# safe-autonomous-systems/fluidgym

Measured on NVIDIA B200. Metric: env-steps/sec (solver steps x envs), higher is better.
Workload: dtype f32

## Files before the change

fluidgym_b200/csrc/piso_b200.cu:

```cuda
#include <cuda_runtime.h>
#include <cooperative_groups.h>
#include <stdint.h>
#include <stdio.h>
#include <stdlib.h>
#include <string.h>
#include <math.h>
#include <new>

#include "fluidgym_b200.h"

namespace cg = cooperative_groups;

static thread_local char g_err[512] = "";
static int set_err(int code, const char *msg, cudaError_t ce = cudaSuccess) {
    if (ce != cudaSuccess) snprintf(g_err, sizeof(g_err), "%s: %s", msg, cudaGetErrorString(ce));
    else snprintf(g_err, sizeof(g_err), "%s", msg);
    return code;
}
extern "C" const char *fgb_last_error(void) { return g_err; }
extern "C" int fgb_version(void) { return 1; }

#define LAUNCH_CHECK(name)                                                       \
    do {                                                                         \
        cudaError_t e_ = cudaGetLastError();                                     \
// ... 1221 lines not shown
            const int nb = ok ? t.nbr[ff * N + g] : -1;
            if (flags & 1) co[k][ff] = (ok && nb >= 0) ? off[(int)t.rev[ff * N + g] * N + nb] : 0.f;
            else co[k][ff] = (ok && nb >= 0) ? off[ff * N + g] : 0.f;
            const int gi = nb >= 0 ? nb : (ok ? g : start);
            const int c = gi / per;
            if (PUSH) na[k][ff] = vs_addr + 4u * (uint32_t)(ok ? t.cg_slot[ff * N + g] : 0);
            else na[k][ff] = mapa_u32(vs_addr + 4u * (uint32_t)(gi - c * per), (uint32_t)c);
        }
    }
    const uint32_t peer_red = mapa_u32(red_addr, (uint32_t)(lane < CS ? lane : 0));
    const uint32_t peer_mb = mapa_u32(mb_addr, (uint32_t)(lane < CS ? lane : 0));
    cluster_sync_all();

    uint32_t rcount = 0;
    uint32_t pphase = 0;
    auto cluster_sum = [&](float a0) -> float {
        const uint32_t w = rcount & 1u, par = (rcount >> 1) & 1u;
#pragma unroll
        for (int o = 16; o > 0; o >>= 1) a0 += __shfl_xor_sync(0xffffffffu, a0, o);
        if (lane < CS) st_async_f32(peer_red + 4u * (w * NP + rank * NW + (uint32_t)warp), a0, peer_mb + 8u * w);
        mbar_wait(mb_addr + 8u * w, par);
        const float *rp = red + w * NP;
        float s0 = 0.f;
#pragma unroll
        for (int q = 0; q < (NP + 31) / 32; ++q) s0 += (lane + 32 * q < NP) ? rp[lane + 32 * q] : 0.f;
#pragma unroll
        for (int o = 16; o > 0; o >>= 1) s0 += __shfl_xor_sync(0xffffffffu, s0, o);
        if (threadIdx.x == 0) mbar_arrive_expect_tx(mb_addr + 8u * w, NP * 4);
        ++rcount;
        return s0;
    };
    auto publish = [&]() {
        __syncthreads();
        if (PUSH) {
            for (int e = threadIdx.x; e < n_exp; e += T) {
                const uint2 ex = exps[e];
                st_async_f32(ex.y, ld_shared_f32(vs_addr + (ex.x & 0xffffffu)), mapa_u32(mb_addr + 16, ex.x >> 24));
            }
        } else if (threadIdx.x < CS) mbar_arrive_remote_release(mapa_u32(mb_addr + 16, threadIdx.x));
    };
    auto acquire_p = [&]() {
        mbar_wait(mb_addr + 16, pphase); pphase ^= 1u;
        if (PUSH && threadIdx.x == 0) mbar_arrive_expect_tx(mb_addr + 16, halo_bytes);
    };
    auto apply = [&](int k) -> float {
        float s = cd[k] * vs[threadIdx.x + k * T];
#pragma unroll
        for (int ff = 0; ff < 4; ++ff) s += co[k][ff] * (PUSH ? ld_shared_f32(na[k][ff]) : ld_dsmem_f32(na[k][ff]));
        return s;
    };
    auto load_f = [&](int k) -> float { const int l = threadIdx.x + k * T; return l < cnt ? f[start + l] : 0.f; };

    float nz = 0.f;
#pragma unroll
    for (int k = 0; k < CPT; ++k) nz += (load_f(k) != 0.f) ? 1.f : 0.f;
    const float nzt = cluster_sum(nz);
    int used = -1; float fin = 0.f;
    if (!(nzt > 0.f)) {
#pragma unroll
        for (int k = 0; k < CPT; ++k) xr[k] = 0.f;
    } else {
        if (!zero_init) {
#pragma unroll
            for (int k = 0; k < CPT; ++k) vs[threadIdx.x + k * T] = xr[k];
            publish(); acquire_p();
#pragma unroll
            for (int k = 0; k < CPT; ++k) rr[k] = load_f(k) - apply(k);
            (void)cluster_sum(0.f);
        } else {
#pragma unroll
            for (int k = 0; k < CPT; ++k) rr[k] = load_f(k);
        }
        float a0 = 0.f;
#pragma unroll
        for (int k = 0; k < CPT; ++k) { const int l = threadIdx.x + k * T; vs[l] = rr[k]; bs[l] = xr[k]; a0 += rr[k] * rr[k]; }
        publish();
        float rho = cluster_sum(a0);
        float bestc = 0.f, lastc = 0.f; int best_it = -1, rising = 0;
        bool take_best = false;
        float pk[CPT], apk[CPT];
        for (int i = 0; i < maxit; ++i) {
            if (reset_steps > 0 && (i + 1) % reset_steps == 0) {
                acquire_p();
                (void)cluster_sum(0.f);
#pragma unroll
                for (int k = 0; k < CPT; ++k) vs[threadIdx.x + k * T] = xr[k];
                publish(); acquire_p();
#pragma unroll
                for (int k = 0; k < CPT; ++k) rr[k] = load_f(k) - apply(k);
                (void)cluster_sum(0.f);
                a0 = 0.f;
#pragma unroll
                for (int k = 0; k < CPT; ++k) { vs[threadIdx.x + k * T] = rr[k]; a0 += rr[k] * rr[k]; }
                publish();
                rho = cluster_sum(a0);
            }
            acquire_p();
            a0 = 0.f;
#pragma unroll
            for (int k = 0; k < CPT; ++k) {
                apk[k] = apply(k);
                pk[k] = vs[threadIdx.x + k * T];
                a0 += pk[k] * apk[k];
            }
            const float pap = cluster_sum(a0);
            const float alpha = rho / pap;
            a0 = 0.f;
#pragma unroll
            for (int k = 0; k < CPT; ++k) {
                xr[k] += alpha * pk[k];
                rr[k] -= alpha * apk[k];
                a0 += rr[k] * rr[k];
            }
            const float rr2 = cluster_sum(a0);
            const float crit = sqrtf(rr2) * norm;
            int stop = isfinite(crit) ? 0 : 1;
            used = i; fin = crit;
            if (!stop) {
                if (i == 0 || crit < bestc) {
                    bestc = crit; best_it = i;
#pragma unroll
                    for (int k = 0; k < CPT; ++k) bs[threadIdx.x + k * T] = xr[k];
                }
                if (i > 0 && crit >= lastc) ++rising; else rising = 0;
                lastc = crit;
                if (crit < tol) stop = 1;
                else if (i == maxit - 1 || rising >= 100) stop = 2;
            }
            asm volatile("" : "+r"(stop));
            if (stop) { take_best = stop == 2; break; }
            const float beta = rr2 / rho;
            rho = rr2;
#pragma unroll
            for (int k = 0; k < CPT; ++k) vs[threadIdx.x + k * T] = rr[k] + beta * pk[k];
            publish();
        }
        if (take_best) {
#pragma unroll
            for (int k = 0; k < CPT; ++k) xr[k] = bs[threadIdx.x + k * T];
            used = best_it; fin = bestc;
        }
    }
    float sx = 0.f;
#pragma unroll
    for (int k = 0; k < CPT; ++k) sx += xr[k];
    const float mean = (flags & 2) ? 0.f : cluster_sum(sx) / (float)N;
    if (mean_out && threadIdx.x == 0 && rank == 0) mean_out[b] = mean;
#pragma unroll
    for (int k = 0; k < CPT; ++k) { const int l = threadIdx.x + k * T; if (l < cnt) xo[start + l] = xr[k] - mean; }
    if (threadIdx.x == 0 && rank == 0) { iters[b * 8 + 2 + slot] = used; resid[b * 8 + 2 + slot] = fin; iter_total[b * 2] += (unsigned long long)(used + 1); }
    cluster_sync_all();
}

template <int T, int CPT, int CS, int MINB>
__global__ void __launch_bounds__(T, MINB) k_cg_strip(Tab t, const float *__restrict__ Poff, const float *__restrict__ Pdiag,
                                                    const float *__restrict__ Rhs, float *__restrict__ Xout,
                                                    int maxit, float tol, int zero_init, int reset_steps, int slot,
                                                    const int32_t *__restrict__ active, int32_t *__restrict__ iters,
                                                    float *__restrict__ resid, unsigned long long *__restrict__ iter_total,
                                                    int flags, float *__restrict__ mean_out, float *__restrict__ best) {
    static_assert(T % 32 == 0, "whole warps only: every warp contributes exactly one partial sum per exchange");
    constexpr int NW = T / 32;
    const int b = blockIdx.x / CS;
    uint32_t rank;
    asm volatile("mov.u32 %0, %%cluster_ctarank;" : "=r"(rank));
    if (active && !active[b]) return;
    extern __shared__ __align__(16) float smem[];
    const int N = t.N, SL = t.st_slots, G = t.st_gmax;
    float4 *co4 = reinterpret_cast<float4 *>(smem);
    float *cdg = smem + 4 * CPT * T;
    float *vs = cdg + CPT * T;
    float *rs = vs + SL;
    float *red = rs + G;
    float *wpart = red + 2 * CS + (2 * CS & 1 ? 1 : 0);
    unsigned long long *mb = (unsigned long long *)(wpart + 2 * NW + (2 * NW & 1 ? 1 : 0));
    uint2 *rex = (uint2 *)(mb + 4);
    uint2 *lex = rex + t.st_remax;
    const float *off = Poff + (size_t)b * 4 * N, *dg = Pdiag + (size_t)b * N, *f = Rhs + (size_t)b * N;
    float *xo = Xout + (size_t)b * N;
    const float norm = 1.0f / sqrtf((float)N);
    const uint32_t red_addr = smem_u32(red), mb_addr = smem_u32(mb), rs_addr = smem_u32(rs);
    const int tid = threadIdx.x, lane = tid & 31, warp = tid >> 5;

    const int4 th0 = reinterpret_cast<const int4 *>(t.st_thread)[((size_t)rank * T + tid) * 2];
    const int4 th1 = reinterpret_cast<const int4 *>(t.st_thread)[((size_t)rank * T + tid) * 2 + 1];
    const int S = th0.y;
    float *vp = vs + th0.x;
    const int re_off = th0.w & 0xffff, re_cnt = (th0.w >> 16) & 0xff;
    const int n_lex = t.st_cnt[4 * rank + 2];
    const float *rgp = rs + th1.y;
    const uint32_t rm = (uint32_t)th1.z;
    const int32_t *cellp = t.st_cell + ((size_t)rank * T + tid) * CPT;
    float *bestp = best + ((size_t)b * CS + rank) * T * CPT + tid;
    const uint32_t bytesA = CS * 4u, bytesB = CS * 4u + 4u * (uint32_t)t.st_cnt[4 * rank];
    if (tid == 0) {
        mbar_init(mb_addr, 1); mbar_init(mb_addr + 8, 1);
        mbar_init(mb_addr + 16, NW); mbar_init(mb_addr + 24, NW);
        asm volatile("fence.mbarrier_init.release.cluster;" ::: "memory");
        mbar_arrive_expect_tx(mb_addr, bytesA);
        mbar_arrive_expect_tx(mb_addr + 8, bytesB);
    }
    for (int e = tid; e < t.st_cnt[4 * rank + 1]; e += T) {
        const int32_t a = t.st_rexp[((size_t)rank * t.st_remax + e) * 2], d = t.st_rexp[((size_t)rank * t.st_remax + e) * 2 + 1];
        rex[e] = make_uint2((uint32_t)a, mapa_u32(rs_addr + 4u * (uint32_t)d, (uint32_t)a >> 8));
    }
    for (int e = tid; e < n_lex; e += T)
        lex[e] = make_uint2((uint32_t)t.st_lexp[((size_t)rank * t.st_lemax + e) * 2], (uint32_t)t.st_lexp[((size_t)rank * t.st_lemax + e) * 2 + 1]);
    for (int i = tid; i < SL + G; i += T) vs[i] = 0.f;

    float x[CPT], r[CPT], ap[CPT];
#pragma unroll
    for (int k = 0; k < CPT; ++k) {
        const int c = cellp[k];
        const bool real = c >= 0;
        const int g = real ? c : (c <= -2 ? -2 - c : 0);
        float co[4];
#pragma unroll
        for (int d = 0; d < 4; ++d) {
            const int ff = (th0.z >> (2 * d)) & 3;
            const int nb = real ? t.nbr[ff * N + g] : -1;
            if (flags & 1) co[d] = nb >= 0 ? off[(int)t.rev[ff * N + g] * N + nb] : 0.f;
            else co[d] = nb >= 0 ? off[ff * N + g] : 0.f;
        }
        co4[k * T + tid] = make_float4(co[0], co[1], co[2], co[3]);
        cdg[k * T + tid] = real ? dg[g] : 0.f;
        x[k] = (c != -1 && !zero_init) ? xo[g] : 0.f;
        r[k] = real ? f[g] : 0.f;
        ap[k] = 0.f;
    }
    const uint32_t peer_red = mapa_u32(red_addr, (uint32_t)(lane < CS ? lane : 0));
    const uint32_t peer_mb = mapa_u32(mb_addr, (uint32_t)(lane < CS ? lane : 0));
    cluster_sync_all();

    uint32_t parA = 0, parB = 0;
    auto exchange = [&](float a0, const uint32_t which, uint32_t &par, const uint32_t bytes) -> float {
#pragma unroll
        for (int o = 16; o > 0; o >>= 1) a0 += __shfl_xor_sync(0xffffffffu, a0, o);
        if (lane == 0) {
            wpart[which * NW + warp] = a0;
            asm volatile("mbarrier.arrive.release.cta.shared::cta.b64 _, [%0];" ::"r"(mb_addr + 16u + 8u * which) : "memory");
        }
        if (warp == 0) {
            mbar_wait_sleep(mb_addr + 16u + 8u * which, par);
            float s1 = lane < NW ? wpart[which * NW + lane] : 0.f;
#pragma unroll
            for (int o = 16; o > 0; o >>= 1) s1 += __shfl_xor_sync(0xffffffffu, s1, o);
            if (lane < CS) st_async_f32(peer_red + 4u * (which * CS + rank), s1, peer_mb + 8u * which);
        }
        mbar_wait_sleep(mb_addr + 8u * which, par); par ^= 1u;
        float s0 = 0.f;
#pragma unroll
        for (int q = 0; q < CS; ++q) s0 += red[which * CS + q];
        if (tid == 0) mbar_arrive_expect_tx(mb_addr + 8u * which, bytes);
        return s0;
    };
    auto row_of = [&](const float (&v)[CPT], int kk) -> float {
        float s = v[0];
#pragma unroll
        for (int k = 1; k < CPT; ++k) s = (kk == k) ? v[k] : s;
        return s;
    };
    auto spmv = [&]() -> float {
        float a0 = 0.f, a1 = 0.f;
        float vsouth = vp[-S], vc = vp[0];
#pragma unroll
        for (int k = 0; k < CPT; ++k) {
            const float *row = vp + k * S;
            const float vnorth = row[S];
            const float4 o = co4[k * T + tid];
            float s = cdg[k * T + tid] * vc;
            s = fmaf(o.x, row[-1], s);
            s = fmaf(o.y, row[1], s);
            s = fmaf(o.z, vsouth, s);
            s = fmaf(o.w, vnorth, s);
            ap[k] = s;
            if (k & 1) a1 = fmaf(vc, s, a1); else a0 = fmaf(vc, s, a0);
            vsouth = vc; vc = vnorth;
        }
        return a0 + a1;
    };
    auto mirror_local_ghosts = [&]() {
        __syncthreads();
        if (n_lex) {
            for (int e = tid; e < n_lex; e += T) { const uint2 ex = lex[e]; vs[ex.y] = vs[ex.x]; }
            __syncthreads();
        }
    };
    auto publish_x = [&]() {
#pragma unroll
        for (int k = 0; k < CPT; ++k) vp[k * S] = x[k];
        mirror_local_ghosts();
    };
    auto new_direction = [&](float beta) {
        if (rm) {
            int n = 0;
#pragma unroll
            for (int k = 0; k < CPT; ++k) if (rm & (1u << k)) r[k] = rgp[n++];
        }
#pragma unroll
        for (int k = 0; k < CPT; ++k) ap[k] = vp[k * S];
#pragma unroll
        for (int k = 0; k < CPT; ++k) vp[k * S] = fmaf(beta, ap[k], r[k]);
        if (rm) {
#pragma unroll
            for (int k = 0; k < CPT; ++k) if (rm & (1u << k)) r[k] = 0.f;
        }
        mirror_local_ghosts();
    };
    auto residual_norm2 = [&]() -> float {
        for (int j = 0; j < re_cnt; ++j) {
            const uint2 ex = rex[re_off + j];
            st_async_f32(ex.y, row_of(r, (int)(ex.x & 0xff)), mapa_u32(mb_addr + 8, ex.x >> 8));
        }
        float a0 = 0.f, a1 = 0.f;
#pragma unroll
        for (int k = 0; k < CPT; k += 2) { a0 = fmaf(r[k], r[k], a0); if (k + 1 < CPT) a1 = fmaf(r[k + 1], r[k + 1], a1); }
        return exchange(a0 + a1, 1u, parB, bytesB);
    };

    float nz = 0.f;
#pragma unroll
    for (int k = 0; k < CPT; ++k) nz += (r[k] != 0.f) ? 1.f : 0.f;
    const float nzt = exchange(nz, 0u, parA, bytesA);
    int used = -1; float fin = 0.f;
    bool solved = false;
    if (!(nzt > 0.f)) {
#pragma unroll
        for (int k = 0; k < CPT; ++k) x[k] = 0.f;
    } else {
        solved = true;
        if (!zero_init) {
            publish_x();
            (void)spmv();
#pragma unroll
            for (int k = 0; k < CPT; ++k) r[k] -= ap[k];
            __syncthreads();
        }
#pragma unroll
        for (int k = 0; k < CPT; ++k) bestp[k * T] = x[k];
        float rho = residual_norm2();
        new_direction(0.f);
        float bestc = 0.f, lastc = 0.f; int best_it = -1, rising = 0;
        bool take_best = false;
        int until_reset = reset_steps > 0 ? reset_steps - 1 : -1;
        for (int i = 0; i < maxit; ++i) {
            if (until_reset == 0) {
                until_reset = reset_steps;
                (void)exchange(0.f, 0u, parA, bytesA);
                publish_x();
                (void)spmv();
#pragma unroll
                for (int k = 0; k < CPT; ++k) { const int c = cellp[k]; r[k] = (c >= 0 ? f[c] : 0.f) - ap[k]; }
                __syncthreads();
                rho = residual_norm2();
                new_direction(0.f);
            }
            --until_reset;
            const float pap = exchange(spmv(), 0u, parA, bytesA);
            const float alpha = rho / pap;
#pragma unroll
            for (int k = 0; k < CPT; ++k) {
                x[k] = fmaf(alpha, vp[k * S], x[k]);
                r[k] = fmaf(-alpha, ap[k], r[k]);
            }
            const float rr2 = residual_norm2();
            const float crit = sqrtf(rr2) * norm;
            int stop = isfinite(crit) ? 0 : 1;
            used = i; fin = crit;
            if (!stop) {
                if (i == 0 || crit < bestc) {
                    bestc = crit; best_it = i;
#pragma unroll
                    for (int k = 0; k < CPT; ++k) bestp[k * T] = x[k];
                }
                if (i > 0 && crit >= lastc) ++rising; else rising = 0;
                lastc = crit;
                if (crit < tol) stop = 1;
                else if (i == maxit - 1 || rising >= 100) stop = 2;
            }
            asm volatile("" : "+r"(stop));
            if (stop) { take_best = stop == 2; break; }
            const float beta = rr2 / rho;
            rho = rr2;
            new_direction(beta);
        }
        if (take_best) {
#pragma unroll
            for (int k = 0; k < CPT; ++k) x[k] = bestp[k * T];
            used = best_it; fin = bestc;
        }
    }
    float mean = 0.f;
    if (solved && !(flags & 2)) {
        float sx = 0.f;
#pragma unroll
        for (int k = 0; k < CPT; ++k) sx += (cellp[k] >= 0) ? x[k] : 0.f;
        mean = exchange(sx, 0u, parA, bytesA) / (float)N;
    }
    if (mean_out && tid == 0 && rank == 0) mean_out[b] = mean;
#pragma unroll
    for (int k = 0; k < CPT; ++k) { const int c = cellp[k]; if (c >= 0) xo[c] = x[k] - mean; }
    if (tid == 0 && rank == 0) { iters[b * 8 + 2 + slot] = used; resid[b * 8 + 2 + slot] = fin; iter_total[b * 2] += (unsigned long long)(used + 1); }
    cluster_sync_all();
}

template <int E> struct EnvTag { static constexpr int value = E; };

template <int T, int CPT, int CS>
__global__ void __launch_bounds__(T, 1) k_cg_strip2(Tab t, const float *__restrict__ Poff, const float *__restrict__ Pdiag,
                                                    const float *__restrict__ Rhs, float *__restrict__ Xout, int B,
                                                    int maxit, float tol, int zero_init, int reset_steps, int slot,
                                                    const int32_t *__restrict__ active, int32_t *__restrict__ iters,
                                                    float *__restrict__ resid, unsigned long long *__restrict__ iter_total,
                                                    int flags, float *__restrict__ mean_out, float *__restrict__ best) {
    static_assert(T % 32 == 0, "whole warps only");
    constexpr int NW = T / 32;
    constexpr uint32_t FULL = 0xffffffffu;
    const int b0 = 2 * (int)(blockIdx.x / CS);
    uint32_t rank;
    asm volatile("mov.u32 %0, %%cluster_ctarank;" : "=r"(rank));
    bool on[2];
    on[0] = !active || active[b0];
    on[1] = b0 + 1 < B && (!active || active[b0 + 1]);
    if (!on[0] && !on[1]) return;
    extern __shared__ __align__(16) float smem[];
    const int N = t.N, SL = t.st_slots, G = t.st_gmax;
    const int ENVF = (5 * CPT * T + SL + G + 2 * CS + 2 * NW + 3) & ~3;
    unsigned long long *mb = (unsigned long long *)(smem + 2 * ENVF);
    unsigned int *cnt = (unsigned int *)(mb + 4);
    uint2 *rex = (uint2 *)(cnt + 4);
    uint2 *lex = rex + t.st_remax;
    const float norm = 1.0f / sqrtf((float)N);
    const uint32_t mb_addr = smem_u32(mb);
    const int tid = threadIdx.x, lane = tid & 31, warp = tid >> 5;

    const int4 th0 = reinterpret_cast<const int4 *>(t.st_thread)[((size_t)rank * T + tid) * 2];
    const int4 th1 = reinterpret_cast<const int4 *>(t.st_thread)[((size_t)rank * T + tid) * 2 + 1];
    const int S = th0.y;
    const int vp_off = 5 * CPT * T + th0.x;
    const int re_off = th0.w & 0xffff, re_cnt = (th0.w >> 16) & 0xff;
    const int n_lex = t.st_cnt[4 * rank + 2];
    const int rg_off = 5 * CPT * T + SL + th1.y;
    const uint32_t rm = (uint32_t)th1.z;
    const int32_t *cellp = t.st_cell + ((size_t)rank * T + tid) * CPT;
    const uint32_t bytesA = CS * 4u, bytesB = CS * 4u + 4u * (uint32_t)t.st_cnt[4 * rank];
    if (tid == 0) {
#pragma unroll
        for (int e = 0; e < 2; ++e) {
            mbar_init(mb_addr + 16u * e, 1); mbar_init(mb_addr + 16u * e + 8u, 1);
            cnt[2 * e] = 0u; cnt[2 * e + 1] = 0u;
        }
        asm volatile("fence.mbarrier_init.release.cluster;" ::: "memory");
#pragma unroll
        for (int e = 0; e < 2; ++e) { mbar_arrive_expect_tx(mb_addr + 16u * e, bytesA); mbar_arrive_expect_tx(mb_addr + 16u * e + 8u, bytesB); }
    }
    {
        const uint32_t rs_addr = smem_u32(smem + 5 * CPT * T + SL);
        for (int e = tid; e < t.st_cnt[4 * rank + 1]; e += T) {
            const int32_t a = t.st_rexp[((size_t)rank * t.st_remax + e) * 2], d = t.st_rexp[((size_t)rank * t.st_remax + e) * 2 + 1];
            rex[e] = make_uint2((uint32_t)a, mapa_u32(rs_addr + 4u * (uint32_t)d, (uint32_t)a >> 8));
        }
    }
    for (int e = tid; e < n_lex; e += T)
        lex[e] = make_uint2((uint32_t)t.st_lexp[((size_t)rank * t.st_lemax + e) * 2], (uint32_t)t.st_lexp[((size_t)rank * t.st_lemax + e) * 2 + 1]);
#pragma unroll
    for (int e = 0; e < 2; ++e)
        for (int i = tid; i < SL + G; i += T) smem[e * ENVF + 5 * CPT * T + i] = 0.f;

    float x[2][CPT], r[2][CPT], ap[2][CPT];
    uint32_t par[2][2] = {{0u, 0u}, {0u, 0u}};
    auto load_env = [&](auto E) {
        constexpr int e = decltype(E)::value;
        const int b = b0 + e;
        const float *off = Poff + (size_t)b * 4 * N, *dg = Pdiag + (size_t)b * N, *f = Rhs + (size_t)b * N;
        const float *xo = Xout + (size_t)b * N;
        float4 *co4 = reinterpret_cast<float4 *>(smem + e * ENVF);
        float *cdg = smem + e * ENVF + 4 * CPT * T;
#pragma unroll
        for (int k = 0; k < CPT; ++k) {
            const int c = cellp[k];
            const bool real = c >= 0;
            const int g = real ? c : (c <= -2 ? -2 - c : 0);
            float co[4];
#pragma unroll
            for (int d = 0; d < 4; ++d) {
                const int ff = (th0.z >> (2 * d)) & 3;
                const int nb = real ? t.nbr[ff * N + g] : -1;
                if (flags & 1) co[d] = nb >= 0 ? off[(int)t.rev[ff * N + g] * N + nb] : 0.f;
                else co[d] = nb >= 0 ? off[ff * N + g] : 0.f;
            }
            co4[k * T + tid] = make_float4(co[0], co[1], co[2], co[3]);
            cdg[k * T + tid] = real ? dg[g] : 0.f;
            x[e][k] = (c != -1 && !zero_init) ? xo[g] : 0.f;
            r[e][k] = real ? f[g] : 0.f;
            ap[e][k] = 0.f;
        }
    };
#pragma unroll
    for (int k = 0; k < CPT; ++k) { x[0][k] = r[0][k] = ap[0][k] = 0.f; x[1][k] = r[1][k] = ap[1][k] = 0.f; }
    if (on[0]) load_env(EnvTag<0>{});
    if (on[1]) load_env(EnvTag<1>{});
    const uint32_t peer_smem = mapa_u32(smem_u32(smem), (uint32_t)(lane < CS ? lane : 0));
    const uint32_t peer_mb = mapa_u32(mb_addr, (uint32_t)(lane < CS ? lane : 0));
    cluster_sync_all();

    auto xstart = [&](auto E, auto W, float a0) {
        constexpr int e = decltype(E)::value;
        constexpr uint32_t which = decltype(W)::value;
        float *red = smem + e * ENVF + 5 * CPT * T + SL + G;
        volatile float *wpart = red + 2 * CS;
#pragma unroll
        for (int o = 16; o > 0; o >>= 1) a0 += __shfl_xor_sync(FULL, a0, o);
        unsigned int last = 0u;
        if (lane == 0) {
            wpart[which * NW + warp] = a0;
            __threadfence_block();
            last = atomicInc(&cnt[2 * e + which], (unsigned int)(NW - 1)) == (unsigned int)(NW - 1);
        }
        last = __shfl_sync(FULL, last, 0);
        if (last) {
            __threadfence_block();
            float s1 = lane < NW ? wpart[which * NW + lane] : 0.f;
#pragma unroll
            for (int o = 16; o > 0; o >>= 1) s1 += __shfl_xor_sync(FULL, s1, o);
            if (lane < CS)
                st_async_f32(peer_smem + 4u * (uint32_t)(e * ENVF + 5 * CPT * T + SL + G + which * CS + rank), s1, peer_mb + 16u * e + 8u * which);
        }
    };
    auto xfinish = [&](auto E, auto W) -> float {
        constexpr int e = decltype(E)::value;
        constexpr uint32_t which = decltype(W)::value;
        const float *red = smem + e * ENVF + 5 * CPT * T + SL + G;
        mbar_wait_sleep(mb_addr + 16u * e + 8u * which, par[e][which]); par[e][which] ^= 1u;
        float s0 = 0.f;
#pragma unroll
        for (int q = 0; q < CS; ++q) s0 += red[which * CS + q];
        if (tid == 0) mbar_arrive_expect_tx(mb_addr + 16u * e + 8u * which, which ? bytesB : bytesA);
        return s0;
    };
    auto spmv = [&](auto E) -> float {
        constexpr int e = decltype(E)::value;
        const float4 *co4 = reinterpret_cast<const float4 *>(smem + e * ENVF);
        const float *cdg = smem + e * ENVF + 4 * CPT * T, *vp = smem + e * ENVF + vp_off;
        float a0 = 0.f, a1 = 0.f;
        float vsouth = vp[-S], vc = vp[0];
#pragma unroll
        for (int k = 0; k < CPT; ++k) {
            const float *row = vp + k * S;
            const float vnorth = row[S];
            const float4 o = co4[k * T + tid];
            float s = cdg[k * T + tid] * vc;
            s = fmaf(o.x, row[-1], s);
            s = fmaf(o.y, row[1], s);
            s = fmaf(o.z, vsouth, s);
            s = fmaf(o.w, vnorth, s);
            ap[e][k] = s;
// ... 1258 lines not shown
            atomicAdd(&Sbvalb[(size_t)b * NB + j], rb * (-(sig * Fb) + dif));
            atomicAdd(&Fbb[(size_t)b * NB + j], -rb * sb[j] * sig);
        }
    }
    fluxes_adjoint(t, g, nb, flb, Ub + (size_t)b * 2 * N, nullptr);
}

__global__ void k_adj_inactive(const int32_t *__restrict__ active, int nc, int n, const float *__restrict__ Uob, float *__restrict__ Ub,
                               const float *__restrict__ Pob, float *__restrict__ Pb, const float *__restrict__ Tob, float *__restrict__ Tb,
                               int nbv, float *__restrict__ Bvb, int nsb, float *__restrict__ Sbb) {
    const int b = blockIdx.y;
    if (active[b]) return;
    const int i = blockIdx.x * blockDim.x + threadIdx.x;
    const size_t nu = (size_t)nc * n;
    if ((size_t)i < nu) Ub[b * nu + i] = Uob[b * nu + i];
    if (i < n) {
        if (Pb) Pb[(size_t)b * n + i] = Pob[(size_t)b * n + i];
        if (Tb) Tb[(size_t)b * n + i] = Tob[(size_t)b * n + i];
    }
    if (i < nbv) Bvb[(size_t)b * nbv + i] = 0.f;
    if (Sbb && i < nsb) Sbb[(size_t)b * nsb + i] = 0.f;
}
static int launch_adj_inactive(const int32_t *active, int B, int nc, int n, const float *uob, float *ub, const float *pob, float *pb,
                               const float *tob, float *tb, int nbv, float *bvb, int nsb, float *sbb, cudaStream_t st) {
    if (!active) return 0;
    int m = nc * n;
    if (nbv > m) m = nbv;
    if (nsb > m) m = nsb;
    k_adj_inactive<<<dim3((unsigned)((m + 255) / 256), (unsigned)B), 256, 0, st>>>(active, nc, n, uob, ub, pob, pb, tob, tb, nbv, bvb, nsb, sbb);
    const cudaError_t ce = cudaGetLastError();
    return ce == cudaSuccess ? 0 : set_err(FGB_E_CUDA, "k_adj_inactive launch", ce);
}

static inline dim3 cell_grid(const fgb_batch *b) { return dim3((b->t.N + 255) / 256, b->B); }
#define STREAM(s) ((cudaStream_t)(s))

static inline void launch_setup_advection(fgb_batch *b, cudaStream_t st, const float *u, const float *ures, const float *bvel, const float *src,
                                          const float *dt, const int32_t *active, int with_matrix) {
    const int ae = b->asm_envs > 1 ? b->asm_envs : 1;
    const dim3 gm((b->t.N + 255) / 256, (b->B + ae - 1) / ae);
    if (ae == 8) k_setup_advection_multi<8><<<gm, 256, 0, st>>>(b->t, b->B, u, ures, bvel, src, dt, active, b->Coff, b->A, b->rhs, with_matrix);
    else if (ae == 4) k_setup_advection_multi<4><<<gm, 256, 0, st>>>(b->t, b->B, u, ures, bvel, src, dt, active, b->Coff, b->A, b->rhs, with_matrix);
    else if (ae == 2) k_setup_advection_multi<2><<<gm, 256, 0, st>>>(b->t, b->B, u, ures, bvel, src, dt, active, b->Coff, b->A, b->rhs, with_matrix);
    else k_setup_advection<<<cell_grid(b), 256, 0, st>>>(b->t, u, ures, bvel, src, dt, active, b->Coff, b->A, b->rhs, with_matrix);
}

extern "C" int fgb_setup_advection(fgb_batch *b, const float *u, const float *ures, const float *bvel, const float *src,
                                   const float *dt, const int32_t *active, fgb_stream_t s) {
    if (!b || !u || !bvel || !dt) return set_err(FGB_E_ARG, "fgb_setup_advection: null argument");
    ProfScope ps(b, CLS_ASM, STREAM(s));
    launch_setup_advection(b, STREAM(s), u, ures ? ures : u, bvel, src, dt, active, 1);
    LAUNCH_CHECK("k_setup_advection");
    return FGB_OK;
}
extern "C" int fgb_solve_advection(fgb_batch *b, int zero_init, const int32_t *active, fgb_stream_t s) {
    if (!b) return set_err(FGB_E_ARG, "fgb_solve_advection: null argument");
    ProfScope ps(b, CLS_BICG, STREAM(s));
    return run_bicgstab<2>(b, b->rhs, b->ures, zero_init, active, STREAM(s));
}
extern "C" int fgb_setup_pressure_matrix(fgb_batch *b, const int32_t *active, fgb_stream_t s) {
    if (!b) return set_err(FGB_E_ARG, "fgb_setup_pressure_matrix: null argument");
    ProfScope ps(b, CLS_ASM, STREAM(s));
    const int ae = b->asm_envs > 1 ? b->asm_envs : 1;
    const dim3 gm((b->t.N + 255) / 256, (b->B + ae - 1) / ae);
    if (ae == 8) k_setup_pressure_matrix_multi<8><<<gm, 256, 0, STREAM(s)>>>(b->t, b->B, b->A, active, b->Poff, b->Pdiag);
    else if (ae == 4) k_setup_pressure_matrix_multi<4><<<gm, 256, 0, STREAM(s)>>>(b->t, b->B, b->A, active, b->Poff, b->Pdiag);
    else if (ae == 2) k_setup_pressure_matrix_multi<2><<<gm, 256, 0, STREAM(s)>>>(b->t, b->B, b->A, active, b->Poff, b->Pdiag);
    else k_setup_pressure_matrix<<<cell_grid(b), 256, 0, STREAM(s)>>>(b->t, b->A, active, b->Poff, b->Pdiag);
    LAUNCH_CHECK("k_setup_pressure_matrix");
    return FGB_OK;
}
extern "C" int fgb_setup_pressure_rhs(fgb_batch *b, const float *u, const float *bvel, const float *src, const float *p_prev,
                                      const float *dt, int with_hbya, const int32_t *active, fgb_stream_t s) {
    if (!b || !bvel) return set_err(FGB_E_ARG, "fgb_setup_pressure_rhs: null argument");
    ProfScope ps(b, CLS_ASM, STREAM(s));
    if (with_hbya) {
        if (!u || !dt) return set_err(FGB_E_ARG, "fgb_setup_pressure_rhs: u/dt required with_hbya");
        b->launches++;
        k_hbya<<<cell_grid(b), 256, 0, STREAM(s)>>>(b->t, u, b->ures, bvel, src, b->Coff, b->A, dt, active, b->hbya);
        LAUNCH_CHECK("k_hbya");
    }
    const int no = b->opt.nonortho && p_prev;
    const int ae = b->asm_envs > 1 ? b->asm_envs : 1;
    const dim3 gm((b->t.N + 255) / 256, (b->B + ae - 1) / ae);
    if (ae == 8) k_pressure_div_multi<8><<<gm, 256, 0, STREAM(s)>>>(b->t, b->B, b->hbya, bvel, p_prev, b->A, active, no, b->div);
    else if (ae == 4) k_pressure_div_multi<4><<<gm, 256, 0, STREAM(s)>>>(b->t, b->B, b->hbya, bvel, p_prev, b->A, active, no, b->div);
    else if (ae == 2) k_pressure_div_multi<2><<<gm, 256, 0, STREAM(s)>>>(b->t, b->B, b->hbya, bvel, p_prev, b->A, active, no, b->div);
    else k_pressure_div<<<cell_grid(b), 256, 0, STREAM(s)>>>(b->t, b->hbya, bvel, p_prev, b->A, active, no, b->div);
    LAUNCH_CHECK("k_pressure_div");
    return FGB_OK;
}

template <int CS, int CPT, int VARIANT>
static int launch_cg_cluster(fgb_batch *b, float *p_out, int zero_init, int reset_steps, int max_iter, int slot,
                             const int32_t *active, cudaStream_t st) {
    constexpr int T = 512;
    const int N = b->t.N;
    const int per = (N + CS - 1) / CS;
    if (per > T * CPT) return 1;
    const size_t smem = ((size_t)2 * T * CPT + (size_t)2 * (T / 32) * CS) * sizeof(float) + 16;
    auto kern = k_cg_cluster<T, CPT, CS, VARIANT>;
    cudaError_t ce = cudaFuncSetAttribute(kern, cudaFuncAttributeMaxDynamicSharedMemorySize, (int)smem);
    if (ce != cudaSuccess) return set_err(FGB_E_CUDA, "cudaFuncSetAttribute(k_cg_cluster)", ce);
    cudaLaunchConfig_t cfg; memset(&cfg, 0, sizeof(cfg));
    cfg.gridDim = dim3(b->B * CS); cfg.blockDim = dim3(T); cfg.dynamicSmemBytes = smem; cfg.stream = st;
    cudaLaunchAttribute attr[1];
    attr[0].id = cudaLaunchAttributeClusterDimension;
    attr[0].val.clusterDim.x = CS; attr[0].val.clusterDim.y = 1; attr[0].val.clusterDim.z = 1;
    cfg.attrs = attr; cfg.numAttrs = 1;
    ce = cudaLaunchKernelEx(&cfg, kern, b->t, (const float *)b->Poff, (const float *)b->Pdiag, (const float *)b->div, p_out,
                            max_iter, b->opt.p_tol, zero_init, reset_steps, slot, active, b->iters, b->resid, b->iter_total);
    if (ce != cudaSuccess) return set_err(FGB_E_CUDA, "cudaLaunchKernelEx(k_cg_cluster)", ce);
    return FGB_OK;
}

template <int CS, int CPT, bool PUSH = false, int T = 512, int MINB = 1>
static int launch_cg_cluster_mb(fgb_batch *b, const float *poff, const float *pdiag, const float *rhs, float *p_out, int zero_init,
                                int reset_steps, int max_iter, int slot, const int32_t *active, int flags, float *mean_out,
                                cudaStream_t st) {
    const int N = b->t.N;
    const int per = (N + CS - 1) / CS;
    if (per > T * CPT) return 1;
    if (PUSH && (!b->t.cg_slot || !b->t.cg_exp || !b->t.cg_cnt || b->t.cg_cs != CS || b->t.cg_pad != T * CPT))
        return set_err(FGB_E_ARG, "cg_impl 6: tables.cg_* (halo plan) missing or built for another cluster size");
    const size_t smem = ((size_t)2 * T * CPT + (size_t)2 * (T / 32) * CS + (PUSH ? (size_t)b->t.cg_hmax : 0)) * sizeof(float) + 4 * 8 + 16 +
                        (PUSH ? (size_t)b->t.cg_emax * 8 : 0);
    if (smem > 227 * 1024) return set_err(FGB_E_ARG, "cg_impl 6: halo plan does not fit in shared memory");
    auto kern = k_cg_cluster_mb<T, CPT, CS, PUSH, MINB>;
    cudaError_t ce = cudaFuncSetAttribute(kern, cudaFuncAttributeMaxDynamicSharedMemorySize, (int)smem);
    if (ce != cudaSuccess) return set_err(FGB_E_CUDA, "cudaFuncSetAttribute(k_cg_cluster_mb)", ce);
    if (CS > 8) {
        ce = cudaFuncSetAttribute(kern, cudaFuncAttributeNonPortableClusterSizeAllowed, 1);
        if (ce != cudaSuccess) return set_err(FGB_E_CUDA, "cudaFuncSetAttribute(k_cg_cluster_mb, non-portable cluster)", ce);
    }
    cudaLaunchConfig_t cfg; memset(&cfg, 0, sizeof(cfg));
    cfg.gridDim = dim3(b->B * CS); cfg.blockDim = dim3(T); cfg.dynamicSmemBytes = smem; cfg.stream = st;
    cudaLaunchAttribute attr[1];
    attr[0].id = cudaLaunchAttributeClusterDimension;
    attr[0].val.clusterDim.x = CS; attr[0].val.clusterDim.y = 1; attr[0].val.clusterDim.z = 1;
    cfg.attrs = attr; cfg.numAttrs = 1;
    ce = cudaLaunchKernelEx(&cfg, kern, b->t, poff, pdiag, rhs, p_out, max_iter, b->opt.p_tol, zero_init, reset_steps, slot, active,
                            b->iters, b->resid, b->iter_total, flags, mean_out);
    if (ce != cudaSuccess) return set_err(FGB_E_CUDA, "cudaLaunchKernelEx(k_cg_cluster_mb)", ce);
    return FGB_OK;
}

template <int T, int CPT, int CS, int MINB>
static int launch_cg_strip(fgb_batch *b, const float *poff, const float *pdiag, const float *rhs, float *p_out, int zero_init,
                           int reset_steps, int max_iter, int slot, const int32_t *active, int flags, float *mean_out,
                           cudaStream_t st) {
    if (b->t.st_cs != CS || b->t.st_T != T || b->t.st_cpt != CPT) return 1;
    if ((size_t)CS * T * CPT > (size_t)KRY_VECS * b->t.N)
        return set_err(FGB_E_ARG, "cg_impl 11: domain too small for the best-iterate scratch (use cg_impl 6)");
    const size_t smem = ((size_t)5 * CPT * T + (size_t)b->t.st_slots + (size_t)b->t.st_gmax + (size_t)2 * CS + 2 * (T / 32) + 2) * sizeof(float) + 4 * 8 +
                        ((size_t)b->t.st_remax + (size_t)b->t.st_lemax) * 8;
    if (smem > 227 * 1024 || (b->t.st_slots & 3) || (b->t.st_gmax & 1))
        return set_err(FGB_E_ARG, "cg_impl 11: strip plan does not fit in shared memory");
    auto kern = k_cg_strip<T, CPT, CS, MINB>;
    cudaError_t ce = cudaFuncSetAttribute(kern, cudaFuncAttributeMaxDynamicSharedMemorySize, (int)smem);
    if (ce != cudaSuccess) return set_err(FGB_E_CUDA, "cudaFuncSetAttribute(k_cg_strip)", ce);
    if (CS > 8) {
        ce = cudaFuncSetAttribute(kern, cudaFuncAttributeNonPortableClusterSizeAllowed, 1);
        if (ce != cudaSuccess) return set_err(FGB_E_CUDA, "cudaFuncSetAttribute(k_cg_strip, non-portable cluster)", ce);
    }
    cudaLaunchConfig_t cfg; memset(&cfg, 0, sizeof(cfg));
    cfg.gridDim = dim3(b->B * CS); cfg.blockDim = dim3(T); cfg.dynamicSmemBytes = smem; cfg.stream = st;
    cudaLaunchAttribute attr[1];
    attr[0].id = cudaLaunchAttributeClusterDimension;
    attr[0].val.clusterDim.x = CS; attr[0].val.clusterDim.y = 1; attr[0].val.clusterDim.z = 1;
    cfg.attrs = attr; cfg.numAttrs = 1;
    ce = cudaLaunchKernelEx(&cfg, kern, b->t, poff, pdiag, rhs, p_out, max_iter, b->opt.p_tol, zero_init, reset_steps, slot, active,
                            b->iters, b->resid, b->iter_total, flags, mean_out, b->kry);
    if (ce != cudaSuccess) return set_err(FGB_E_CUDA, "cudaLaunchKernelEx(k_cg_strip)", ce);
    return FGB_OK;
}

template <int T, int CPT, int MINB>
static int cg_strip_cs(fgb_batch *b, const float *poff, const float *pdiag, const float *rhs, float *p_out, int zero_init,
                       int reset_steps, int max_iter, int slot, const int32_t *active, int flags, float *mean_out, cudaStream_t st) {
    int rc = launch_cg_strip<T, CPT, 1, MINB>(b, poff, pdiag, rhs, p_out, zero_init, reset_steps, max_iter, slot, active, flags, mean_out, st);
    if (rc == 1) rc = launch_cg_strip<T, CPT, 2, MINB>(b, poff, pdiag, rhs, p_out, zero_init, reset_steps, max_iter, slot, active, flags, mean_out, st);
    if (rc == 1) rc = launch_cg_strip<T, CPT, 4, MINB>(b, poff, pdiag, rhs, p_out, zero_init, reset_steps, max_iter, slot, active, flags, mean_out, st);
    if (rc == 1) rc = launch_cg_strip<T, CPT, 8, MINB>(b, poff, pdiag, rhs, p_out, zero_init, reset_steps, max_iter, slot, active, flags, mean_out, st);
    if (rc == 1) rc = launch_cg_strip<T, CPT, 16, MINB>(b, poff, pdiag, rhs, p_out, zero_init, reset_steps, max_iter, slot, active, flags, mean_out, st);
    return rc;
}
static int cg_strip_any(fgb_batch *b, const float *poff, const float *pdiag, const float *rhs, float *p_out, int zero_init,
                        int reset_steps, int max_iter, int slot, const int32_t *active, int flags, float *mean_out, cudaStream_t st) {
    int rc = cg_strip_cs<480, 17, 1>(b, poff, pdiag, rhs, p_out, zero_init, reset_steps, max_iter, slot, active, flags, mean_out, st);
    if (rc == 1) rc = cg_strip_cs<256, 17, 2>(b, poff, pdiag, rhs, p_out, zero_init, reset_steps, max_iter, slot, active, flags, mean_out, st);
    if (rc == 1) rc = cg_strip_cs<896, 9, 1>(b, poff, pdiag, rhs, p_out, zero_init, reset_steps, max_iter, slot, active, flags, mean_out, st);
    if (rc == 1) rc = cg_strip_cs<640, 13, 1>(b, poff, pdiag, rhs, p_out, zero_init, reset_steps, max_iter, slot, active, flags, mean_out, st);
    if (rc == 1) rc = cg_strip_cs<320, 13, 2>(b, poff, pdiag, rhs, p_out, zero_init, reset_steps, max_iter, slot, active, flags, mean_out, st);
    return rc;
}


template <int T, int CPT, int CS>
static int launch_cg_strip2(fgb_batch *b, const float *poff, const float *pdiag, const float *rhs, float *p_out, int zero_init,
                            int reset_steps, int max_iter, int slot, const int32_t *active, int flags, float *mean_out,
                            cudaStream_t st) {
    if (b->t.st_cs != CS || b->t.st_T != T || b->t.st_cpt != CPT) return 1;
    if ((size_t)CS * T * CPT > (size_t)KRY_VECS * b->t.N)
        return set_err(FGB_E_ARG, "cg_impl 12: domain too small for the best-iterate scratch (use cg_impl 6)");
    const size_t envf = ((size_t)5 * CPT * T + (size_t)b->t.st_slots + (size_t)b->t.st_gmax + (size_t)2 * CS + 2 * (T / 32) + 3) & ~(size_t)3;
    const size_t smem = 2 * envf * sizeof(float) + 4 * 8 + 4 * 4 + ((size_t)b->t.st_remax + (size_t)b->t.st_lemax) * 8;
    if (smem > 227 * 1024 || (b->t.st_slots & 3) || (b->t.st_gmax & 1))
        return set_err(FGB_E_ARG, "cg_impl 12: strip plan does not fit in shared memory");
    auto kern = k_cg_strip2<T, CPT, CS>;
    cudaError_t ce = cudaFuncSetAttribute(kern, cudaFuncAttributeMaxDynamicSharedMemorySize, (int)smem);
    if (ce != cudaSuccess) return set_err(FGB_E_CUDA, "cudaFuncSetAttribute(k_cg_strip2)", ce);
    if (CS > 8) {
        ce = cudaFuncSetAttribute(kern, cudaFuncAttributeNonPortableClusterSizeAllowed, 1);
        if (ce != cudaSuccess) return set_err(FGB_E_CUDA, "cudaFuncSetAttribute(k_cg_strip2, non-portable cluster)", ce);
    }
    cudaLaunchConfig_t cfg; memset(&cfg, 0, sizeof(cfg));
    cfg.gridDim = dim3(((b->B + 1) / 2) * CS); cfg.blockDim = dim3(T); cfg.dynamicSmemBytes = smem; cfg.stream = st;
    cudaLaunchAttribute attr[1];
    attr[0].id = cudaLaunchAttributeClusterDimension;
    attr[0].val.clusterDim.x = CS; attr[0].val.clusterDim.y = 1; attr[0].val.clusterDim.z = 1;
    cfg.attrs = attr; cfg.numAttrs = 1;
    ce = cudaLaunchKernelEx(&cfg, kern, b->t, poff, pdiag, rhs, p_out, b->B, max_iter, b->opt.p_tol, zero_init, reset_steps, slot, active,
                            b->iters, b->resid, b->iter_total, flags, mean_out, b->kry);
    if (ce != cudaSuccess) return set_err(FGB_E_CUDA, "cudaLaunchKernelEx(k_cg_strip2)", ce);
    return FGB_OK;
}
static int cg_strip2_any(fgb_batch *b, const float *poff, const float *pdiag, const float *rhs, float *p_out, int zero_init,
                         int reset_steps, int max_iter, int slot, const int32_t *active, int flags, float *mean_out, cudaStream_t st) {
    int rc = launch_cg_strip2<480, 9, 2>(b, poff, pdiag, rhs, p_out, zero_init, reset_steps, max_iter, slot, active, flags, mean_out, st);
    if (rc == 1) rc = launch_cg_strip2<480, 9, 4>(b, poff, pdiag, rhs, p_out, zero_init, reset_steps, max_iter, slot, active, flags, mean_out, st);
    if (rc == 1) rc = launch_cg_strip2<480, 9, 8>(b, poff, pdiag, rhs, p_out, zero_init, reset_steps, max_iter, slot, active, flags, mean_out, st);
    return rc;
}

static inline bool uses_halo_plan(int cg_impl) { return cg_impl == 6 || cg_impl == 11 || cg_impl == 12; }

static int cg_cluster_mb_any(fgb_batch *b, const float *poff, const float *pdiag, const float *rhs, float *p_out, int zero_init,
                             int reset_steps, int max_iter, int slot, const int32_t *active, int flags, float *mean_out, cudaStream_t st) {
    if (b->opt.cg_impl == 12 && b->t.st_thread && b->t.st_cell && b->t.st_rexp && b->t.st_lexp && b->t.st_cnt) {
        const int rc = cg_strip2_any(b, poff, pdiag, rhs, p_out, zero_init, reset_steps, max_iter, slot, active, flags, mean_out, st);
        if (rc == 1) return set_err(FGB_E_ARG, "cg_impl 12: no k_cg_strip2 instantiation for the shape (st_T, st_cpt, st_cs) of this strip plan");
        return rc;
    }
    if (b->opt.cg_impl == 11 && b->t.st_thread && b->t.st_cell && b->t.st_rexp && b->t.st_lexp && b->t.st_cnt) {
        const int rc = cg_strip_any(b, poff, pdiag, rhs, p_out, zero_init, reset_steps, max_iter, slot, active, flags, mean_out, st);
        if (rc == 1) return set_err(FGB_E_ARG, "cg_impl 11: no k_cg_strip instantiation for the shape (st_T, st_cpt, st_cs) of this strip plan");
        return rc;
    }
    if (b->opt.cg_impl == 8) {
        int rc = launch_cg_cluster_mb<2, 7, true, 256, 2>(b, poff, pdiag, rhs, p_out, zero_init, reset_steps, max_iter, slot, active, flags, mean_out, st);
        if (rc == 1) rc = launch_cg_cluster_mb<4, 7, true, 256, 2>(b, poff, pdiag, rhs, p_out, zero_init, reset_steps, max_iter, slot, active, flags, mean_out, st);
        if (rc == 1) rc = launch_cg_cluster_mb<8, 7, true, 256, 2>(b, poff, pdiag, rhs, p_out, zero_init, reset_steps, max_iter, slot, active, flags, mean_out, st);
        if (rc == 1) rc = launch_cg_cluster_mb<16, 7, true, 256, 2>(b, poff, pdiag, rhs, p_out, zero_init, reset_steps, max_iter, slot, active, flags, mean_out, st);
        return rc;
    }
    if (b->opt.cg_impl == 7) {
        int rc = launch_cg_cluster_mb<2, 12, true, 256>(b, poff, pdiag, rhs, p_out, zero_init, reset_steps, max_iter, slot, active, flags, mean_out, st);
        if (rc == 1) rc = launch_cg_cluster_mb<4, 14, true, 256>(b, poff, pdiag, rhs, p_out, zero_init, reset_steps, max_iter, slot, active, flags, mean_out, st);
        if (rc == 1) rc = launch_cg_cluster_mb<8, 14, true, 256>(b, poff, pdiag, rhs, p_out, zero_init, reset_steps, max_iter, slot, active, flags, mean_out, st);
        if (rc == 1) rc = launch_cg_cluster_mb<16, 12, true, 256>(b, poff, pdiag, rhs, p_out, zero_init, reset_steps, max_iter, slot, active, flags, mean_out, st);
        return rc;
    }
    if (uses_halo_plan(b->opt.cg_impl)) {
        int rc = launch_cg_cluster_mb<2, 6, true>(b, poff, pdiag, rhs, p_out, zero_init, reset_steps, max_iter, slot, active, flags, mean_out, st);
        if (rc == 1) rc = launch_cg_cluster_mb<4, 7, true>(b, poff, pdiag, rhs, p_out, zero_init, reset_steps, max_iter, slot, active, flags, mean_out, st);
        if (rc == 1) rc = launch_cg_cluster_mb<8, 7, true>(b, poff, pdiag, rhs, p_out, zero_init, reset_steps, max_iter, slot, active, flags, mean_out, st);
        if (rc == 1) rc = launch_cg_cluster_mb<16, 6, true>(b, poff, pdiag, rhs, p_out, zero_init, reset_steps, max_iter, slot, active, flags, mean_out, st);
        return rc;
    }
    int rc = launch_cg_cluster_mb<2, 6>(b, poff, pdiag, rhs, p_out, zero_init, reset_steps, max_iter, slot, active, flags, mean_out, st);
    if (rc == 1) rc = launch_cg_cluster_mb<4, 7>(b, poff, pdiag, rhs, p_out, zero_init, reset_steps, max_iter, slot, active, flags, mean_out, st);
    if (rc == 1) rc = launch_cg_cluster_mb<8, 7>(b, poff, pdiag, rhs, p_out, zero_init, reset_steps, max_iter, slot, active, flags, mean_out, st);
    if (rc == 1) rc = launch_cg_cluster_mb<16, 6>(b, poff, pdiag, rhs, p_out, zero_init, reset_steps, max_iter, slot, active, flags, mean_out, st);
    return rc;
}

template <int CS, int CPT, int MINB>
static int launch_cg_smem(fgb_batch *b, float *p_out, int zero_init, int reset_steps, int max_iter, int slot,
                          const int32_t *active, cudaStream_t st) {
    constexpr int T = 512;
    const int N = b->t.N;
    const int per = (N + CS - 1) / CS;
    if (per > T * CPT) return 1;
    const size_t smem = ((size_t)6 * T * CPT + (size_t)2 * (T / 32) * CS) * sizeof(float) + 3 * 8 + 16;
    auto kern = k_cg_smem<T, CPT, CS, MINB>;
    cudaError_t ce = cudaFuncSetAttribute(kern, cudaFuncAttributeMaxDynamicSharedMemorySize, (int)smem);
    if (ce != cudaSuccess) return set_err(FGB_E_CUDA, "cudaFuncSetAttribute(k_cg_smem)", ce);
    cudaLaunchConfig_t cfg; memset(&cfg, 0, sizeof(cfg));
    cfg.gridDim = dim3(b->B * CS); cfg.blockDim = dim3(T); cfg.dynamicSmemBytes = smem; cfg.stream = st;
    cudaLaunchAttribute attr[1];
    attr[0].id = cudaLaunchAttributeClusterDimension;
    attr[0].val.clusterDim.x = CS; attr[0].val.clusterDim.y = 1; attr[0].val.clusterDim.z = 1;
    cfg.attrs = attr; cfg.numAttrs = 1;
    ce = cudaLaunchKernelEx(&cfg, kern, b->t, (const float *)b->Poff, (const float *)b->Pdiag, (const float *)b->div, p_out,
                            max_iter, b->opt.p_tol, zero_init, reset_steps, slot, active, b->iters, b->resid, b->iter_total);
    if (ce != cudaSuccess) return set_err(FGB_E_CUDA, "cudaLaunchKernelEx(k_cg_smem)", ce);
    return FGB_OK;
}

static int solve_pressure_slot(fgb_batch *b, float *p_out, int zero_init, int reset_steps, int max_iter, int slot,
                               const int32_t *active, fgb_stream_t s) {
    if (!b || !p_out) return set_err(FGB_E_ARG, "fgb_solve_pressure: null argument");
    const int mean_slot = slot < 0 ? 7 : (slot > 7 ? 7 : slot);
    if (slot < 0 || slot > 5) slot = 5;
    ProfScope ps(b, CLS_CG, STREAM(s));
    if (b->opt.cg_impl == 4) {
        int rc = launch_cg_smem<1, 12, 1>(b, p_out, zero_init, reset_steps, max_iter, slot, active, STREAM(s));
        if (rc == 1) rc = launch_cg_smem<2, 14, 1>(b, p_out, zero_init, reset_steps, max_iter, slot, active, STREAM(s));
        if (rc == 1) rc = launch_cg_smem<4, 12, 1>(b, p_out, zero_init, reset_steps, max_iter, slot, active, STREAM(s));
        if (rc <= 0) return rc;
    }
    if (b->opt.cg_impl == 5) {
        int rc = launch_cg_smem<2, 6, 2>(b, p_out, zero_init, reset_steps, max_iter, slot, active, STREAM(s));
// ... 514 lines not shown
```

Measured before the change: 48170.

## Store CG strip stencil coefficients in tensor memory instead of shared memory

Moves the per-thread stencil coefficients (four off-diagonals plus diagonal) of the strip CG kernel out of shared memory and into TMEM, allocated per CTA with tcgen05.alloc. The SpMV reads them back with chunked tcgen05.ld, issuing the next chunk's load before the current chunk's arithmetic. This frees shared memory and shared-memory bandwidth for the vector halo and reduction buffers. The host side shrinks the smem request, sets a smem carveout, and checks occupancy against the 512 TMEM columns per SM. The cost is TMEM alloc/dealloc per launch and a possible limit on co-resident CTAs.

```diff
diff --git a/fluidgym_b200/csrc/piso_b200.cu b/fluidgym_b200/csrc/piso_b200.cu
--- a/fluidgym_b200/csrc/piso_b200.cu
+++ b/fluidgym_b200/csrc/piso_b200.cu
@@ -1397,6 +1397,21 @@
     cluster_sync_all();
 }
 
+__device__ __forceinline__ void tmem_fence_before() { asm volatile("tcgen05.fence::before_thread_sync;" ::: "memory"); }
+__device__ __forceinline__ void tmem_fence_after() { asm volatile("tcgen05.fence::after_thread_sync;" ::: "memory"); }
+__device__ __forceinline__ void tmem_st1(uint32_t taddr, float v) {
+    asm volatile("tcgen05.st.sync.aligned.32x32b.x1.b32 [%0], {%1};" ::"r"(taddr), "r"(__float_as_uint(v)) : "memory");
+}
+__device__ __forceinline__ void tmem_ld4(uint32_t taddr, uint32_t (&v)[4]) {
+    asm volatile("tcgen05.ld.sync.aligned.32x32b.x4.b32 {%0, %1, %2, %3}, [%4];"
+                 : "=r"(v[0]), "=r"(v[1]), "=r"(v[2]), "=r"(v[3]) : "r"(taddr));
+}
+__device__ __forceinline__ void tmem_wait_ld(uint32_t (&v)[4]) {
+    asm volatile("tcgen05.wait::ld.sync.aligned;" : "+r"(v[0]), "+r"(v[1]), "+r"(v[2]), "+r"(v[3]));
+}
+template <int MINB> __host__ __device__ constexpr int cg_strip_tmem_cols() { return MINB == 1 ? 512 : 256; }
+template <int CPT> __host__ __device__ constexpr int cg_strip_tmem_row_cols() { return (5 * CPT + 7) / 8 * 8; }
+
 template <int T, int CPT, int CS, int MINB>
 __global__ void __launch_bounds__(T, MINB) k_cg_strip(Tab t, const float *__restrict__ Poff, const float *__restrict__ Pdiag,
                                                     const float *__restrict__ Rhs, float *__restrict__ Xout,
@@ -1406,15 +1421,27 @@
                                                     int flags, float *__restrict__ mean_out, float *__restrict__ best) {
     static_assert(T % 32 == 0, "whole warps only: every warp contributes exactly one partial sum per exchange");
     constexpr int NW = T / 32;
+    constexpr int TCOLS = cg_strip_tmem_cols<MINB>(), CR = cg_strip_tmem_row_cols<CPT>(), NCH = CR / 4;
+    static_assert((NW + 3) / 4 * CR <= TCOLS, "stencil coefficients exceed the TMEM allocation");
+    static_assert(MINB * TCOLS <= 512, "co-resident CTAs would need more than the SM's 512 TMEM columns");
     const int b = blockIdx.x / CS;
     uint32_t rank;
     asm volatile("mov.u32 %0, %%cluster_ctarank;" : "=r"(rank));
     if (active && !active[b]) return;
     extern __shared__ __align__(16) float smem[];
+    __shared__ uint32_t tmem_slot;
+    const int tid = threadIdx.x, lane = tid & 31, warp = tid >> 5;
+    if (warp == 0) {
+        asm volatile("tcgen05.alloc.cta_group::1.sync.aligned.shared::cta.b32 [%0], %1;" ::"r"(smem_u32(&tmem_slot)), "r"(TCOLS) : "memory");
+        asm volatile("tcgen05.relinquish_alloc_permit.cta_group::1.sync.aligned;" ::: "memory");
+    }
+    tmem_fence_before();
+    __syncthreads();
+    tmem_fence_after();
+    const uint32_t tbase = tmem_slot;
+    const uint32_t tm = tbase + ((uint32_t)(32 * (warp & 3)) << 16) + (uint32_t)((warp >> 2) * CR);
     const int N = t.N, SL = t.st_slots, G = t.st_gmax;
-    float4 *co4 = reinterpret_cast<float4 *>(smem);
-    float *cdg = smem + 4 * CPT * T;
-    float *vs = cdg + CPT * T;
+    float *vs = smem;
     float *rs = vs + SL;
     float *red = rs + G;
     float *wpart = red + 2 * CS + (2 * CS & 1 ? 1 : 0);
@@ -1425,7 +1452,6 @@
     float *xo = Xout + (size_t)b * N;
     const float norm = 1.0f / sqrtf((float)N);
     const uint32_t red_addr = smem_u32(red), mb_addr = smem_u32(mb), rs_addr = smem_u32(rs);
-    const int tid = threadIdx.x, lane = tid & 31, warp = tid >> 5;
 
     const int4 th0 = reinterpret_cast<const int4 *>(t.st_thread)[((size_t)rank * T + tid) * 2];
     const int4 th1 = reinterpret_cast<const int4 *>(t.st_thread)[((size_t)rank * T + tid) * 2 + 1];
@@ -1467,12 +1493,14 @@
             if (flags & 1) co[d] = nb >= 0 ? off[(int)t.rev[ff * N + g] * N + nb] : 0.f;
             else co[d] = nb >= 0 ? off[ff * N + g] : 0.f;
         }
-        co4[k * T + tid] = make_float4(co[0], co[1], co[2], co[3]);
-        cdg[k * T + tid] = real ? dg[g] : 0.f;
+#pragma unroll
+        for (int d = 0; d < 4; ++d) tmem_st1(tm + 5 * k + d, co[d]);
+        tmem_st1(tm + 5 * k + 4, real ? dg[g] : 0.f);
         x[k] = (c != -1 && !zero_init) ? xo[g] : 0.f;
         r[k] = real ? f[g] : 0.f;
         ap[k] = 0.f;
     }
+    asm volatile("tcgen05.wait::st.sync.aligned;" ::: "memory");
     const uint32_t peer_red = mapa_u32(red_addr, (uint32_t)(lane < CS ? lane : 0));
     const uint32_t peer_mb = mapa_u32(mb_addr, (uint32_t)(lane < CS ? lane : 0));
     cluster_sync_all();
@@ -1506,21 +1534,30 @@
         return s;
     };
     auto spmv = [&]() -> float {
+        uint32_t cb[NCH][4];
+        tmem_ld4(tm, cb[0]);
         float a0 = 0.f, a1 = 0.f;
         float vsouth = vp[-S], vc = vp[0];
-#pragma unroll
-        for (int k = 0; k < CPT; ++k) {
-            const float *row = vp + k * S;
-            const float vnorth = row[S];
-            const float4 o = co4[k * T + tid];
-            float s = cdg[k * T + tid] * vc;
-            s = fmaf(o.x, row[-1], s);
-            s = fmaf(o.y, row[1], s);
-            s = fmaf(o.z, vsouth, s);
-            s = fmaf(o.w, vnorth, s);
-            ap[k] = s;
-            if (k & 1) a1 = fmaf(vc, s, a1); else a0 = fmaf(vc, s, a0);
-            vsouth = vc; vc = vnorth;
+        tmem_wait_ld(cb[0]);
+#pragma unroll
+        for (int c = 0; c < NCH; ++c) {
+            if (c + 1 < NCH) tmem_ld4(tm + 4 * (c + 1), cb[c + 1]);
+#pragma unroll
+            for (int k = 0; k < CPT; ++k) {
+                if ((5 * k + 4) / 4 != c) continue;
+                auto cf = [&](int d) { const int j = 5 * k + d; return __uint_as_float(cb[j / 4][j % 4]); };
+                const float *row = vp + k * S;
+                const float vnorth = row[S];
+                float s = cf(4) * vc;
+                s = fmaf(cf(0), row[-1], s);
+                s = fmaf(cf(1), row[1], s);
+                s = fmaf(cf(2), vsouth, s);
+                s = fmaf(cf(3), vnorth, s);
+                ap[k] = s;
+                if (k & 1) a1 = fmaf(vc, s, a1); else a0 = fmaf(vc, s, a0);
+                vsouth = vc; vc = vnorth;
+            }
+            if (c + 1 < NCH) tmem_wait_ld(cb[c + 1]);
         }
         return a0 + a1;
     };
@@ -1646,7 +1683,12 @@
 #pragma unroll
     for (int k = 0; k < CPT; ++k) { const int c = cellp[k]; if (c >= 0) xo[c] = x[k] - mean; }
     if (tid == 0 && rank == 0) { iters[b * 8 + 2 + slot] = used; resid[b * 8 + 2 + slot] = fin; iter_total[b * 2] += (unsigned long long)(used + 1); }
+    tmem_fence_before();
     cluster_sync_all();
+    if (warp == 0) {
+        tmem_fence_after();
+        asm volatile("tcgen05.dealloc.cta_group::1.sync.aligned.b32 %0, %1;" ::"r"(tbase), "r"(TCOLS) : "memory");
+    }
 }
 
 template <int E> struct EnvTag { static constexpr int value = E; };
@@ -3211,13 +3253,22 @@
     if (b->t.st_cs != CS || b->t.st_T != T || b->t.st_cpt != CPT) return 1;
     if ((size_t)CS * T * CPT > (size_t)KRY_VECS * b->t.N)
         return set_err(FGB_E_ARG, "cg_impl 11: domain too small for the best-iterate scratch (use cg_impl 6)");
-    const size_t smem = ((size_t)5 * CPT * T + (size_t)b->t.st_slots + (size_t)b->t.st_gmax + (size_t)2 * CS + 2 * (T / 32) + 2) * sizeof(float) + 4 * 8 +
+    const size_t smem = ((size_t)b->t.st_slots + (size_t)b->t.st_gmax + (size_t)2 * CS + 2 * (T / 32) + 2) * sizeof(float) + 4 * 8 +
                         ((size_t)b->t.st_remax + (size_t)b->t.st_lemax) * 8;
     if (smem > 227 * 1024 || (b->t.st_slots & 3) || (b->t.st_gmax & 1))
         return set_err(FGB_E_ARG, "cg_impl 11: strip plan does not fit in shared memory");
     auto kern = k_cg_strip<T, CPT, CS, MINB>;
     cudaError_t ce = cudaFuncSetAttribute(kern, cudaFuncAttributeMaxDynamicSharedMemorySize, (int)smem);
     if (ce != cudaSuccess) return set_err(FGB_E_CUDA, "cudaFuncSetAttribute(k_cg_strip)", ce);
+    const size_t pct = (MINB * (smem + 1024 + 16) * 100 + 228 * 1024 - 1) / (228 * 1024);
+    const int carve = pct > 100 ? 100 : (int)pct;
+    ce = cudaFuncSetAttribute(kern, cudaFuncAttributePreferredSharedMemoryCarveout, carve);
+    if (ce != cudaSuccess) return set_err(FGB_E_CUDA, "cudaFuncSetAttribute(k_cg_strip, carve-out)", ce);
+    int occ = 0;
+    ce = cudaOccupancyMaxActiveBlocksPerMultiprocessor(&occ, kern, T, smem);
+    if (ce != cudaSuccess) return set_err(FGB_E_CUDA, "cudaOccupancyMaxActiveBlocksPerMultiprocessor(k_cg_strip)", ce);
+    if (occ * cg_strip_tmem_cols<MINB>() > 512)
+        return set_err(FGB_E_ARG, "cg_impl 11: co-resident k_cg_strip CTAs would need more than 512 TMEM columns per SM");
     if (CS > 8) {
         ce = cudaFuncSetAttribute(kern, cudaFuncAttributeNonPortableClusterSizeAllowed, 1);
         if (ce != cudaSuccess) return set_err(FGB_E_CUDA, "cudaFuncSetAttribute(k_cg_strip, non-portable cluster)", ce);
```

Result: faster. 55960 (median of 6 runs) (+16.2%).
